# koskja/linalg-solver

Measured on AMD Instinct MI355X. Metric: fp64_lu_gflops, higher is better.
Workload: dtype f64; 1 GPU; 8192x8192 f64 LU with partial pivoting (getrf), u11 generator, resident in HBM; n=8192, nb=128, panel_mode=4, lookahead=1, parallelism=single GPU, resident_inputs=189

## Files before the change

linalg_solver_amd/csrc/common.h:

```cpp
#pragma once
#include <hip/hip_runtime.h>
#include <stdint.h>
#include <stdio.h>
#include <string>
#include <vector>

#include "../../include/lsx.h"

#ifdef LSX_TSTAMP
static __device__ long long *lsx_ts_buf;
struct TsScope {
    int id;
    __device__ void put(int tag) {
        long long *b = lsx_ts_buf;
        const int i = atomicAdd((int *)b, 1);
        if (i < (1 << 20)) { b[1 + 2 * i] = tag; b[2 + 2 * i] = wall_clock64(); }
    }
    __device__ TsScope(int id_) : id(id_) { if (lsx_ts_buf && threadIdx.x == 0 && blockIdx.x == 0 && blockIdx.y == 0) put(id); }
    __device__ ~TsScope() { if (lsx_ts_buf && threadIdx.x == 0) put(id | 0x100); }
};
#define LSX_TS(id) TsScope ts_scope_(id)
#define LSX_TS_SETTER(name) extern "C" void lsx_ts_set_##name(long long *p) { (void)hipMemcpyToSymbol(HIP_SYMBOL(lsx_ts_buf), &p, sizeof p); }
#else
#define LSX_TS(id)
#define LSX_TS_SETTER(name)
#endif

namespace lsx {

void set_error(const char *fmt, ...);

#define LSX_HIP(call)                                                                     \
    do {                                                                                  \
        hipError_t e_ = (call);                                                           \
        if (e_ != hipSuccess) {                                                           \
            lsx::set_error("%s failed: %s (%s:%d)", #call, hipGetErrorString(e_), __FILE__, \
                           __LINE__);                                                     \
            return LSX_ERR_HIP;                                                           \
        }                                                                                 \
    } while (0)

#define LSX_TRY(call)              \
    do {                           \
        int r_ = (call);           \
        if (r_ != LSX_OK) return r_; \
    } while (0)

#define LSX_ARG(cond)                                                     \
    do {                                                                  \
        if (!(cond)) {                                                    \
            lsx::set_error("bad argument: %s (%s:%d)", #cond, __FILE__, __LINE__); \
            return LSX_ERR_ARG;                                           \
        }                                                                 \
    } while (0)

struct ProfEvent {
    hipEvent_t a, b;
    int bucket;
};

struct Prof {
    unsigned mask = 0;
    int sample = 1;
    long long seen[LSX_PROF_NBUCKETS] = {0};
    std::vector<ProfEvent> pending;
    std::vector<hipEvent_t> pool;
    double ms[LSX_PROF_NBUCKETS] = {0};
    long long launches[LSX_PROF_NBUCKETS] = {0};
    double flops[LSX_PROF_NBUCKETS] = {0};
    double bytes[LSX_PROF_NBUCKETS] = {0};
};

}

struct DevBuf { void *p = nullptr; size_t bytes = 0; };

struct lsx_handle_s {
    int device = 0;
    int num_cu = 256;
    hipStream_t own_stream = nullptr;
    hipStream_t stream = nullptr;
    hipStream_t side_stream = nullptr;
    hipEvent_t ev_panel = nullptr, ev_next = nullptr, ev_start = nullptr, ev_done = nullptr;
    lsx::Prof prof;
    int nb = 128;
    int kblock = 1;
    int panel_mode = 4;
    int lookahead = 1;
    int lookahead_min = 0;
    int panel_rt = 4;
    int panel_nt = 0;
    int trsv_mode = 2;
    int gemm_stagger = 0;
    int gemm_waves = 0;
    int getri_pairs = 1;
    int left_per_step = 1;
    int chain_fused = 1;
    int chain_wait_limit = 1 << 21;
    int x_events = 0;
    int panel_debug = 0;
    int getri_plain = 0;
    int rref_first_fast = 1;
    int rref_blocked = 1;
    int getrs_t_blocked_min = 64;
    int gesvdj_max_sweeps = 30;
    int syevj_max_sweeps = 60;
    int potrs_few_max = 0;
    int lauum_descending = 0;
    int potri_order = 0;
    int gemm_no_tiles32 = 0;
    int gemm_queue_test = 0;
    int xrows_limit = 0;
    int hybrid_off = 0;
    int panel_spin_limit = 1 << 20;
    int spin_limit = 1 << 20;
    int rref_first_used = 0;
    int gecon_solves = 0;
    int gerfs_steps = 0;
    int gerfs_solves = 0;
    int getrs_t_path = 0;
    int potrs_path = 0;
    int potri_tiles = 0;
    int pocon_solves = 0;
    int porfs_steps = 0;
    int porfs_solves = 0;
    int gesvdj_sweeps = 0;
    int gesvdj_rotations = 0;
    int syevj_sweeps = 0;
    int syevj_rotations = 0;
    int panel_fallbacks = 0;
    DevBuf staging;
    DevBuf tinv;
    DevBuf rhs_work;
    DevBuf mixed_resid;
    DevBuf getri_work;
    DevBuf rref_first;
    DevBuf cond;
    DevBuf refine;
    DevBuf equil;
    DevBuf qr_work;
    DevBuf svd_work;
    DevBuf eig_work;
    DevBuf xchg;
    unsigned xchg_epoch = 0;
    DevBuf moves_all;
    DevBuf scratch;
    void *moves_buf[2] = {nullptr, nullptr};
    void *moves_api = nullptr;
    bool moves_api_valid = false;
    int *dev_status = nullptr;
};

namespace lsx {

struct OnStream {
    lsx_handle_t h; hipStream_t keep;
    OnStream(lsx_handle_t h_, hipStream_t s) : h(h_), keep(h_->stream) { h->stream = s; }
    ~OnStream() { h->stream = keep; }
};

struct GemmPlan {
    int kshift = 0;
    bool mfma_only = false;
    int *col0_static = nullptr;
    int *counters = nullptr;
    const int *avoid_word = nullptr;
    int *pass_word = nullptr;
    int *col0 = nullptr;
};
struct GemmDone {
    bool queued = false;
    bool col0_complete = false;
    int col0_tiles = 0;
};

struct PanelArgs {
    int mode, nt, rt;
    void *list;
    void *area; size_t area_bytes; bool cleared = false;
    int *xcc_word = nullptr;
    bool listed = false;
    PanelArgs(lsx_handle_t h, void *list_) : mode(h->panel_mode), nt(h->panel_nt), rt(h->panel_rt), list(list_), area(h->scratch.p), area_bytes(h->scratch.bytes) {}
};

int reserve(lsx_handle_t h, DevBuf &b, size_t need, bool *fresh = nullptr);
struct Carver {
    char *base;
    size_t off = 0;
    explicit Carver(void *b) : base((char *)b) {}
    template <typename U> U *take(size_t count) {
        off = (off + 255) & ~(size_t)255;
        U *p = base ? (U *)(base + off) : nullptr;
        off += count * sizeof(U);
        return p;
    }
};
template <class F> size_t carve_bytes(F &&layout) {
    Carver count(nullptr);
    layout(count);
    return count.off;
}
template <class F> int carve(lsx_handle_t h, DevBuf &b, F &&layout, bool *fresh = nullptr) {
    LSX_TRY(reserve(h, b, carve_bytes(layout), fresh));
    Carver c(b.p);
    layout(c);
    return LSX_OK;
}
template <class F> int carve_in(void *area, size_t bytes, const char *who, F &&layout) {
    Carver c(area);
    layout(c);
    if (area && c.off <= bytes) return LSX_OK;
    set_error("%s: needs %zu bytes of scratch, was handed %zu", who, c.off, bytes);
    return LSX_ERR_INTERNAL;
}
template <class F> size_t max_over_heights(int m, bool every, F &&bytes) {
    size_t need = 0;
    for (int mm = m; mm > 0; mm = (mm - 1) / 64 * 64) {
        const size_t b = bytes(mm);
        if (every && !b) return 0;
        if (b > need) need = b;
    }
    return need;
}
int ensure_getrf_workspace(lsx_handle_t h, int n, size_t elem);
int panel_xcd_first(lsx_handle_t h, int m, int jb, double *P, int ldp, int row0, int col0, int32_t *d_ipiv, int *d_info, double tol,
                    PanelArgs &pa);
template <typename T>
int launch_gather_pivot_cols(lsx_handle_t h, int m, int r, int row_lo, const T *src, int lds, const int32_t *d_pivots, T *dst, int ldd);
template <typename T>
int launch_rref_finish(lsx_handle_t h, int m, int bar, T *W, int ldw, const int32_t *d_pivots, int rank);
template <typename T>
int rref_blocked(lsx_handle_t h, int m, int n, int bar, T *W, int ldw, int32_t *d_pivots, int *d_rank, double tol, int pivot_rule);

struct ProfScope {
    lsx_handle_t h;
    hipStream_t st;
    int idx = -1;
    ProfScope(lsx_handle_t h_, int bucket, double flops = 0, double bytes = 0);
    ~ProfScope();
};

template <typename T>
struct Real;
template <>
struct Real<double> {
    static constexpr double eps = 2.220446049250313e-16;
};
template <>
struct Real<float> {
    static constexpr float eps = 1.1920929e-07f;
};

template <typename T>
__device__ __forceinline__ T fast_recip(T x) {
    if (sizeof(T) == 8) {
        double r = __builtin_amdgcn_rcp((double)x);
        r = r * (2.0 - (double)x * r);
        r = r * (2.0 - (double)x * r);
        return (T)r;
    }
    float r = __builtin_amdgcn_rcpf((float)x);
    r = r * (2.0f - (float)x * r);
    return (T)r;
}

template <typename T>
struct PivotRecip {
    T c, rinv;
    __device__ __forceinline__ T apply(T a) const { return (a * c) * rinv; }
};
template <typename T>
__device__ __forceinline__ PivotRecip<T> pivot_recip(T p) {
    const T safmin = sizeof(T) == 8 ? (T)0x1p-1022 : (T)0x1p-126f;
    const T c = (p < T(0) ? -p : p) < safmin ? (sizeof(T) == 8 ? (T)0x1p64 : (T)0x1p32f) : T(1);
    return PivotRecip<T>{c, fast_recip<T>(p * c)};
}


template <typename T>
int launch_fill(lsx_handle_t h, int kind, uint64_t seed, int m, int n, T *A, int lda, int row_off,
                int col_off);
template <typename T>
int launch_gemm_sub(lsx_handle_t h, int m, int n, int k, const T *A, int lda, const T *B, int ldb,
                    T *C, int ldc, const GemmPlan &plan = GemmPlan(), GemmDone *done = nullptr);
template <typename T>
int launch_gemm_acc(lsx_handle_t h, int plus, int m, int n, int k, const T *A, int lda, const T *B, int ldb,
                    T *C, int ldc, const GemmPlan &plan = GemmPlan(), GemmDone *done = nullptr);
template <typename T>
int launch_gemm_tn_acc(lsx_handle_t h, int mode, int m, int n, int k, const T *A, int lda, const T *B, int ldb, T *C,
                       int ldc, int bucket = LSX_PROF_GEMM);
template <typename T>
int launch_syrk_tn_sub(lsx_handle_t h, int n, int k, const T *A, int lda, T *C, int ldc);
template <typename T>
int launch_gemm_tn_sub(lsx_handle_t h, int m, int n, int k, const T *A, int lda, const T *B, int ldb, T *C, int ldc);
template <typename T>
int launch_lauum_tn(lsx_handle_t h, int n, const T *V, int ldv, T *C, int ldc, int order, bool descending);
int launch_rref_trace(lsx_handle_t h, int m, int n, int bar, double *R, int ldr, unsigned char *Tm,
                      int32_t *d_pivots, int32_t *d_steps, int max_steps, double *d_snaps,
                      unsigned char *d_snap_t, int max_snaps, int *d_out);
template <typename T>
int launch_panel(lsx_handle_t h, int m, int jb, T *P, int ldp, int row0, int32_t *d_ipiv,
                 int *d_info, PanelArgs &pa);
size_t panel_scratch_bytes(lsx_handle_t h, int mode, int nt, int rt, int m, size_t elem);
size_t panel_pipe_area_bytes(lsx_handle_t h, int mode, int nt, int rt, int m, bool for_driver = true);
size_t panel_x_area_bytes(lsx_handle_t h, int mode, int m, size_t elem, bool for_driver = true);
template <typename T>
int launch_laswp(lsx_handle_t h, int ncols, T *A, int lda, int row0, int jb, const int32_t *d_ipiv);
template <typename T>
int launch_laswp_moves(lsx_handle_t h, const int2 *moves, int ncols, T *A, int lda, int row0);
template <typename T>
int launch_laswp_left_all(lsx_handle_t h, T *A, int lda, int k0, int nb, int nsteps, const void *lists);
int launch_gate(lsx_handle_t h, const int *word, int target);
int launch_wait_count(lsx_handle_t h, const int *word, int target, int *info);
int launch_resid_mixed(lsx_handle_t h, int n, int nrhs, const float *A, int lda, const float *B, int ldb, const double *X,
                       int ldx, float *R, int ldr);
int launch_refine_apply(lsx_handle_t h, int n, int nrhs, int init, const float *D, int ldd, double *X, int ldx, float *Xf,
                        int ldf, double *d_out2);
template <typename T>
int diag_chain_head(lsx_handle_t h, int jb, const T *Tm, int ldt, T *Tinv, int ncols, T *A, int lda, int row0,
                    const void *moves);
template <typename T>
int launch_laswp_moves_around(lsx_handle_t h, const int2 *moves, int n, T *A, int lda, int row0, int hole_at, int hole_w);
template <typename T>
int launch_trtri(lsx_handle_t h, int lower, int jb, const T *Tm, int ldt, T *Tinv);
template <typename T>
int launch_chain_head(lsx_handle_t h, const int2 *moves, int *info, int jb, const T *Tm, int ldt, T *Tinv, int ncols, T *A,
                      int lda, int row0, const int *wait_word = nullptr, int wait_target = 0);
// ... 149 lines not shown
```

linalg_solver_amd/csrc/kernels_panel_x.hip:

```cpp
#include <algorithm>
#include <type_traits>

#include "common.h"
#include "panel_xchg.h"

namespace lsx {

constexpr int PX_WC = 8;
constexpr int PX_NT = 64 * (128 / PX_WC);
constexpr int PX_REC = 128;
constexpr int PX_NONE = 0x7fffffff;
#ifndef LSX_PX_SEG
#define LSX_PX_SEG -1
#endif
#define PX_MARK(k)                                                                  \
    if (LSX_PX_SEG >= 0) {                                                          \
        if (LSX_PX_SEG == (k)) seg_t0 = __builtin_amdgcn_s_memtime();               \
        if (LSX_PX_SEG + 1 == (k)) seg_acc += __builtin_amdgcn_s_memtime() - seg_t0; \
    }

__device__ __forceinline__ int argmax64_fast(unsigned khi, unsigned klo, int idx) {
    const unsigned mhi = rows_max_u32<4>(row16_max_u32(khi), 0);
    const bool top = (khi == mhi) & (idx != PX_NONE);
    const unsigned long long mask = __builtin_amdgcn_ballot_w64(top);
    if (mask == 0ull) return PX_NONE;
    if ((mask & (mask - 1ull)) == 0ull)
        return __builtin_amdgcn_readlane(idx, __builtin_amdgcn_readfirstlane(__builtin_ctzll(mask)));
    const unsigned mlo = rows_max_u32<4>(row16_max_u32(top ? klo : 0u), 0);
    return rows_min_i32<4>(row16_min_i32((top & (klo == mlo)) ? idx : PX_NONE), 0);
}

template <typename T>
__device__ __forceinline__ unsigned long long value_bits(T v) {
    if (sizeof(T) == 8) return (unsigned long long)__double_as_longlong((double)v);
    return (unsigned long long)__float_as_uint((float)v);
}
template <typename T>
__device__ __forceinline__ T bits_value(unsigned lo, unsigned hi) {
    if (sizeof(T) == 8) return (T)__longlong_as_double((long long)(((unsigned long long)hi << 32) | lo));
    return (T)__uint_as_float(lo);
}

template <typename T, int RT, bool DBG, bool XCD, bool FIRST = false>
__device__ __forceinline__ void panel_x_body(const int G, const int g, int m, int jb, T *__restrict__ P, int ldp,
                                             int row0, int col0, int32_t *__restrict__ ipiv,
                                             int *__restrict__ info, char *rec, XGran *far, int *status,
                                             unsigned long long *dbg, int2 *__restrict__ moves, const int spin_limit,
                                             const double tol = -1.0) {
    constexpr int NT = PX_NT, WC = PX_WC;
    constexpr int NW = NT / 64;
    constexpr int RB = 64 * RT;
    constexpr int NONE = PX_NONE;
    __shared__ T s_l[2][RB];
    __shared__ __attribute__((aligned(16))) int4 s_info[2];
    __shared__ int s_cl2;
    __shared__ int s_hist[PC_COLS], s_topid[PC_COLS], s_postop[PC_COLS];
    __shared__ int s_order[RB];
    __shared__ __attribute__((aligned(16))) T s_stage[NW][WC];

    if (info && *info < 0) return;
    const int tid = threadIdx.x, lane = tid & 63, wave = tid >> 6;
    const int base = g * RB;
    const int c0 = WC * wave;
    const bool has_cols = c0 < jb;
    const int nown = (jb + WC - 1) / WC;

    unsigned long long seg[8] = {0, 0, 0, 0, 0, 0, 0, 0};
    unsigned long long seg_t0 = 0, seg_acc = 0;
    unsigned long long tlast = 0;
#define STAMP(i)                                                              \
    if (DBG && LSX_PX_SEG < 0) {                                              \
        const unsigned long long tn_ = __builtin_amdgcn_s_memrealtime();      \
        seg[i] += tn_ - tlast;                                                \
        tlast = tn_;                                                          \
    }

    const __amdgpu_buffer_rsrc_t r_rec = __builtin_amdgcn_make_buffer_rsrc(rec, 0, 2 * G * PX_REC, 0x00020000);
    const __amdgpu_buffer_rsrc_t r_far =
        __builtin_amdgcn_make_buffer_rsrc(far, 0, 4 * G * PC_COLS * (int)sizeof(XGran), 0x00020000);
#define d_rec r_rec
#define d_far r_far

    T a[RT][WC];
    typedef T v2t __attribute__((ext_vector_type(2)));
    const bool wide = (jb == PC_COLS) && ((size_t)P % 16 == 0) && (ldp % 2 == 0);
    if (wide) {
#pragma unroll
        for (int r = 0; r < RT; ++r) {
            const int gi = base + 64 * r + lane;
            const T *src = P + (size_t)(gi < m ? gi : 0) * ldp + c0;
#pragma unroll
            for (int c = 0; c < WC; c += 2) {
                const v2t v = *(const v2t *)(src + c);
                a[r][c] = gi < m ? v[0] : T(0);
                a[r][c + 1] = gi < m ? v[1] : T(0);
            }
        }
    } else {
#pragma unroll
        for (int r = 0; r < RT; ++r) {
            const int gi = base + 64 * r + lane;
            const T *src = P + (size_t)gi * ldp + c0;
#pragma unroll
            for (int c = 0; c < WC; ++c) a[r][c] = (gi < m && c0 + c < jb) ? src[c] : T(0);
        }
    }
    for (int t = tid; t < PC_COLS; t += NT) { s_topid[t] = t; s_postop[t] = t; }
    for (int t = tid; t < RB; t += NT) s_order[t] = -1;
    unsigned frozen = 0;
#pragma unroll
    for (int r = 0; r < RT; ++r)
        if (base + 64 * r + lane >= m) frozen |= 1u << r;
    int pos[FIRST ? RT : 1];
    if (FIRST) {
#pragma unroll
        for (int r = 0; r < RT; ++r) pos[r] = base + 64 * r + lane;
    }
    constexpr unsigned EMASK = FIRST ? 0xffu : 0x7fffffffu;
    auto track_swap = [&](const int j, const int win, const int wpos) __attribute__((always_inline)) {
        if (FIRST) {
#pragma unroll
            for (int r = 0; r < RT; ++r)
                if (pos[r] == j && base + 64 * r + lane != win) pos[r] = wpos;
        }
    };
    bool failed = false;
    u4 hA = u4{0u, 0u, 0u, 0u}, hB = u4{0u, 0u, 0u, 0u};
    __builtin_amdgcn_s_waitcnt(0x0F70);
    __syncthreads();

    auto replay = [&](int jj) __attribute__((always_inline)) {
        const int c = s_hist[jj] & 0x3fffffff;
        const bool zero_piv = (s_hist[jj] >> 30) & 1;
        const int p = (c < jb) ? s_postop[c] : c;
        const int d = s_topid[jj];
        if (p != jj) {
            s_topid[jj] = c;
            if (p < jb) s_topid[p] = d;
            s_postop[d] = p;
            if (c < jb) s_postop[c] = jj;
        }
        if (g == 0) {
            ipiv[jj] = row0 + p;
            if (zero_piv && info && *info == 0) *info = col0 + jj + 1;
        }
    };

    auto shot_async = [&](u4 &h, const int jn) __attribute__((always_inline)) {
        const int off = ((jn & 1) * G + (lane < G ? lane : 0)) * PX_REC;
        asm volatile("buffer_load_dwordx4 %0, %1, %2, 0 offen sc1" : "+v"(h) : "v"(off), "s"(d_rec));
    };
    auto wait_a = [&]() __attribute__((always_inline)) { asm volatile("s_waitcnt vmcnt(1)" : "+v"(hA), "+v"(hB)); };
    auto wait_b = [&]() __attribute__((always_inline)) { asm volatile("s_waitcnt vmcnt(0)" : "+v"(hA), "+v"(hB)); };
    auto store16 = [&](const unsigned lo, const unsigned hi, const unsigned z, const unsigned w, const int off,
                       const __amdgpu_buffer_rsrc_t &desc) __attribute__((always_inline)) {
#define LSX_ST16(R0, R1, R2, R3, POL)                                                                                   \
    asm volatile("v_mov_b32 v" #R0 ", %0\n\tv_mov_b32 v" #R1 ", %1\n\tv_mov_b32 v" #R2 ", %2\n\tv_mov_b32 v" #R3 ", %3\n\t"    \
                 "buffer_store_dwordx4 v[" #R0 ":" #R3 "], %4, %5, 0 offen" POL "\n\ts_nop 1"                             \
                 : : "v"(lo), "v"(hi), "s"(z), "v"(w), "v"(off), "s"(desc) : "v" #R0, "v" #R1, "v" #R2, "v" #R3)
        if (WC == 8) {
            if (XCD) LSX_ST16(124, 125, 126, 127, ""); else LSX_ST16(124, 125, 126, 127, " sc1");
        } else {
            if (XCD) LSX_ST16(252, 253, 254, 255, ""); else LSX_ST16(252, 253, 254, 255, " sc1");
        }
#undef LSX_ST16
    };
    auto store_header = [&](const int jn, const double val, const int row, const bool neg, const int rpos = 0)
                            __attribute__((always_inline)) {
        store16((unsigned)__double2loint(val), (unsigned)__double2hiint(val),
                (unsigned)__builtin_amdgcn_readfirstlane(row),
                (unsigned)(jn + 1) | (neg ? 0x80000000u : 0u) | (FIRST ? ((unsigned)rpos << 8) : 0u),
                ((jn & 1) * G + g) * PX_REC, d_rec);
    };
    auto store_gran = [&](const __amdgpu_buffer_rsrc_t &desc, const int off, const T v, const int jn) __attribute__((always_inline)) {
        unsigned lo, hi;
        if (sizeof(T) == 8) { lo = (unsigned)__double2loint((double)v); hi = (unsigned)__double2hiint((double)v); }
        else { lo = __float_as_uint((float)v); hi = 0u; }
        store16(lo, hi, (unsigned)(jn + 1), 0u, off, desc);
    };
    auto choose_and_announce = [&](auto CNt, const int jn) __attribute__((always_inline)) -> int {
        constexpr int CN = decltype(CNt)::value;
        double nv = -1.0;
        int ni = NONE;
        int np = NONE;
#pragma unroll
        for (int r = 0; r < RT; ++r) {
            const double av = fabs((double)a[r][CN]);
            bool better;
            if (FIRST) better = (((frozen >> r) & 1u) == 0u) & (av > tol) & (pos[r] < np);
            else better = (((frozen >> r) & 1u) == 0u) & (av > nv);
            nv = better ? av : nv;
            ni = better ? base + 64 * r + lane : ni;
            if (FIRST) np = better ? pos[r] : np;
        }
        const unsigned long long kb = (ni != NONE) ? (unsigned long long)__double_as_longlong(nv) : 0ull;
        const int win = FIRST ? argmax64_fast((ni != NONE) ? (unsigned)(0x7fffffff - np) : 0u, 0u, ni)
                              : argmax64_fast((unsigned)(kb >> 32), (unsigned)kb, ni);
        const bool have = win != NONE;
        const int cl = have ? win - base : -1;
        if (have) {
            if (lane == (cl & 63)) {
                const int ck = cl >> 6;
                const int roff = ((jn & 1) * G + g) * PX_REC;
#pragma unroll
                for (int k = 0; k < RT; ++k)
                    if (ck == k) {
                        store_header(jn, fabs((double)a[k][CN]), win, a[k][CN] < T(0), FIRST ? pos[k] : 0);
#pragma unroll
                        for (int c = (CN & 7) + 1; c < 8; ++c)
                            store_gran(d_rec, roff + 16 * c, a[k][(CN & 8) + c], jn);
                    }
            }
        } else if (lane == 0) {
            store_header(jn, 0.0, -1, false);
        }
        return cl;
    };
    const unsigned stage_addr = (unsigned)(unsigned long long)(T __attribute__((address_space(3))) *)&s_stage[wave][0];
    auto publish_far = [&](auto CLOt, auto NCt, const int jn, const int cl_) __attribute__((always_inline)) {
        constexpr int CLO = decltype(CLOt)::value, NC = decltype(NCt)::value;
        const int cl = __builtin_amdgcn_readfirstlane(cl_);
        if (cl < 0 || !has_cols) return;
        if (lane == (cl & 63)) {
            const int ck = cl >> 6;
#pragma unroll
            for (int k = 0; k < RT; ++k)
                if (ck == k) {
#pragma unroll
                    for (int c = 0; c < NC; ++c) {
                        if (sizeof(T) == 8)
                            asm volatile("ds_write_b64 %0, %1 offset:%2" : : "v"(stage_addr), "v"(a[k][CLO + c]), "n"(8 * c) : "memory");
                        else
                            asm volatile("ds_write_b32 %0, %1 offset:%2" : : "v"(stage_addr), "v"(a[k][CLO + c]), "n"(4 * c) : "memory");
                    }
                }
        }
        const int q = lane & (NC - 1);
        unsigned lo, hi = 0u;
        if (sizeof(T) == 8) {
            double v;
            asm volatile("ds_read_b64 %0, %1\n\ts_waitcnt lgkmcnt(0)" : "=v"(v) : "v"(stage_addr + 8u * q) : "memory");
            lo = (unsigned)__double2loint(v); hi = (unsigned)__double2hiint(v);
        } else {
            asm volatile("ds_read_b32 %0, %1\n\ts_waitcnt lgkmcnt(0)" : "=v"(lo) : "v"(stage_addr + 4u * q) : "memory");
        }
        if (lane < NC)
            store16(lo, hi, (unsigned)(jn + 1), 0u, (((jn & 3) * G + g) * PC_COLS + c0 + CLO + q) * (int)sizeof(XGran), d_far);
    };
    auto far_update = [&](auto CLOt, auto NCt, const int j, const int bg) __attribute__((always_inline)) -> bool {
        constexpr int CLO = decltype(CLOt)::value, NC = decltype(NCt)::value;
        const int off = (((j & 3) * G + bg) * PC_COLS + c0 + CLO + (lane & (NC - 1))) * (int)sizeof(XGran);
        u4 v;
        int spins = failed ? spin_limit : 0;
        for (;;) {
            v = __builtin_amdgcn_raw_buffer_load_b128(r_far, off, opaque_zero(), 16);
            if (!__any(v.z != (unsigned)(j + 1))) break;
            if (++spins > spin_limit) return false;
        }
        T l[RT];
#pragma unroll
        for (int r = 0; r < RT; ++r) l[r] = s_l[j & 1][64 * r + lane];
        const T un = -bits_value<T>(v.x, v.y);
        asm volatile("s_nop 1" : : "v"(un));
#pragma unroll
        for (int c = 0; c < NC; ++c) {
#pragma unroll
            for (int r = 0; r < RT; ++r) {
                if (sizeof(T) == 8)
                    asm volatile("v_fmac_f64_dpp %0, %1, %2 row_newbcast:%3 row_mask:0xf bank_mask:0xf"
                                 : "+v"(a[r][CLO + c]) : "v"(un), "v"(l[r]), "n"(c));
                else
                    asm volatile("v_fmac_f32_dpp %0, %1, %2 row_newbcast:%3 row_mask:0xf bank_mask:0xf"
                                 : "+v"(a[r][CLO + c]) : "v"(un), "v"(l[r]), "n"(c));
            }
        }
        return true;
    };
    typedef std::integral_constant<int, 0> I0;
    typedef std::integral_constant<int, 8> I8;
    typedef std::integral_constant<int, WC> IWC;
    auto follow = [&](const int j, const int ow) __attribute__((always_inline)) {
        const int par = j & 1;
        const bool stamp = DBG && wave == ow + 1;
        if (stamp) tlast = __builtin_amdgcn_s_memrealtime();
        __syncthreads();
        if (stamp) STAMP(4)
        const int4 inf = s_info[par];
        const int wrow = inf.x;
        const bool act = (inf.y & 1) != 0;
        failed |= (inf.y & 2) != 0;
        const bool valid = wrow >= 0;
        const int bg = valid ? wrow / RB : 0;
        if (wave == (ow == 0 ? NW - 1 : 0) && lane == 63) {
            s_hist[j] = valid ? (wrow | (act ? 0 : (1 << 30))) : j;
            if (j > 0) replay(j - 1);
            if (valid && bg == g) s_order[wrow - base] = j;
        }
        if (valid && bg == g) {
            const int wl = wrow - base;
            if ((wl & 63) == lane) frozen |= 1u << (wl >> 6);
        }
        if (valid) track_swap(j, wrow, inf.w);
        bool ok = true;
        if (act && wave > ow && has_cols) ok = far_update(I0{}, IWC{}, j, bg);
        if (stamp) STAMP(5)
        if (!ok && !failed) {
            failed = true;
            if (lane == 0) atomicExch(status, 1);
        }
        if (j + 1 < jb) {
            if ((j & 7) < 7) {
                if (wave > ow) publish_far(I0{}, IWC{}, j + 1, inf.z);
            } else {
                const bool hand_over = (j & (WC - 1)) == WC - 1;
                if (hand_over && wave == ow + 1) {
                    __builtin_amdgcn_s_setprio(3);
                    const int cl = choose_and_announce(I0{}, j + 1);
                    if (lane == 0) s_cl2 = cl;
                    shot_async(hA, j + 1);
                }
                __syncthreads();
                const int nown_ = hand_over ? ow + 1 : ow;
                if (hand_over && wave == ow + 1) {
                    if constexpr (WC == 16) publish_far(I8{}, I8{}, j + 1, s_cl2);
                    shot_async(hB, j + 1);
                }
                else if (wave > nown_) publish_far(I0{}, IWC{}, j + 1, s_cl2);
            }
        }
        if (stamp) STAMP(6)
    };

    auto own = [&](auto CJt, const int j) __attribute__((always_inline)) {
        constexpr int CJ = decltype(CJt)::value;
        constexpr int JC = CJ & 7;
        constexpr int CB = CJ & 8;
        constexpr bool FIRSTB = WC == 16 && CJ < 8;
        constexpr bool NEAR = JC < 7;
        const int par = j & 1;
        const bool more = j + 1 < jb;
        if (DBG && CJ == 0) tlast = __builtin_amdgcn_s_memrealtime();
        PX_MARK(0)
        bool failed_now = failed;
        bool pend = lane < G;
        unsigned hlo = 0u, hhi = 0u, hneg = 0u;
        int hrow = NONE;
        int hpos = 0;
        auto absorb = [&](const u4 &h) __attribute__((always_inline)) {
            const bool ok = pend & ((h.w & EMASK) == (unsigned)(j + 1));
            hlo = ok ? h.x : hlo;
            hhi = ok ? h.y : hhi;
            hneg = ok ? (h.w >> 31) : hneg;
            if (FIRST) hpos = ok ? (int)((h.w >> 8) & 0x3fffu) : hpos;
            hrow = ok ? ((int)h.z >= 0 ? (int)h.z : NONE) : hrow;
            pend = ok ? false : pend;
        };
        constexpr bool TWO = !FIRSTB || JC == 0;
        if (TWO) wait_a(); else wait_b();
        PX_MARK(1)
        absorb(hA);
        if (__any(pend)) {
            if (TWO) { wait_b(); absorb(hB); }
            int spins = failed ? spin_limit : 0;
            while (__any(pend)) {
                if (++spins > spin_limit) { failed_now = true; break; }
                const u4 h = __builtin_amdgcn_raw_buffer_load_b128(
                    r_rec, (par * G + (lane < G ? lane : 0)) * PX_REC, opaque_zero(), 16);
                absorb(h);
            }
        }
        const bool hv = hrow != NONE;
        const int win = FIRST ? argmax64_fast(hv ? (unsigned)(0x7fffffff - hpos) : 0u, 0u, hrow)
                              : argmax64_fast(hv ? hhi : 0u, hv ? hlo : 0u, hrow);
        const bool valid = (win != NONE) & !failed_now;
        const int bg = valid ? win / RB : 0;
        const int wpos = FIRST ? __builtin_amdgcn_readlane(hpos, bg) : 0;
        const unsigned plo = (unsigned)__builtin_amdgcn_readlane((int)hlo, bg);
        const unsigned phi = (unsigned)__builtin_amdgcn_readlane((int)hhi, bg);
        const bool pneg = __builtin_amdgcn_readlane((int)hneg, bg) != 0;
        const double pabs = __longlong_as_double((long long)(((unsigned long long)phi << 32) | plo));
        PX_MARK(2)
        STAMP(0)
        const bool act = valid & (pabs != 0.0);
        const bool fetch = NEAR && more && act;
        u4 nq = u4{0u, 0u, 0u, 0u};
        const int noff = (par * G + bg) * PX_REC + 16 * (lane & 7);
        if (fetch) nq = __builtin_amdgcn_raw_buffer_load_b128(r_rec, noff, opaque_zero(), 16);
        PivotRecip<T> rinv = act ? pivot_recip<T>((T)pabs) : PivotRecip<T>{T(1), T(0)};
        if (pneg) rinv.rinv = -rinv.rinv;
        if (valid && bg == g) {
            const int wl = win - base;
            if ((wl & 63) == lane) frozen |= 1u << (wl >> 6);
        }
        if (valid) track_swap(j, win, wpos);
        T l[RT];
#pragma unroll
        for (int r = 0; r < RT; ++r) {
            const T v = rinv.apply(a[r][CJ]);
            l[r] = ((frozen >> r) & 1u) ? T(0) : v;
            s_l[par][64 * r + lane] = l[r];
            a[r][CJ] = (act & (((frozen >> r) & 1u) == 0u)) ? l[r] : a[r][CJ];
        }
        PX_MARK(3)
        wait_b();
        bool upd = false;
        if (fetch) {
            int spins = 0;
            for (;;) {
                const int q = lane & 7;
                if (!__any((q > JC) & (nq.z != (unsigned)(j + 1)))) break;
                if (++spins > spin_limit) { failed_now = true; break; }
                nq = __builtin_amdgcn_raw_buffer_load_b128(r_rec, noff, opaque_zero(), 16);
            }
            upd = !failed_now;
        }
        STAMP(1)
        PX_MARK(4)
        if (upd) {
            const T un = -bits_value<T>(nq.x, nq.y);
            asm volatile("s_nop 1" : : "v"(un));
#pragma unroll
            for (int c = JC + 1; c < 8; ++c) {
#pragma unroll
                for (int r = 0; r < RT; ++r) {
                    if (sizeof(T) == 8)
                        asm volatile("v_fmac_f64_dpp %0, %1, %2 row_newbcast:%3 row_mask:0xf bank_mask:0xf"
                                     : "+v"(a[r][CB + c]) : "v"(un), "v"(l[r]), "n"(c));
                    else
                        asm volatile("v_fmac_f32_dpp %0, %1, %2 row_newbcast:%3 row_mask:0xf bank_mask:0xf"
                                     : "+v"(a[r][CB + c]) : "v"(un), "v"(l[r]), "n"(c));
                }
            }
        }
        PX_MARK(5)
        int cl = -1;
        if (NEAR && more) cl = choose_and_announce(std::integral_constant<int, (CJ < WC - 1 ? CJ + 1 : WC - 1)>{}, j + 1);
        PX_MARK(6)
        const bool act2 = act & !failed_now;
        if (lane == 0) s_info[par] = make_int4(valid ? win : -1, (act2 ? 1 : 0) | (failed_now ? 2 : 0), cl, wpos);
        if (failed_now && !failed) {
            failed = true;
            if (lane == 0) atomicExch(status, 1);
        }
        if (NEAR && more) shot_async(hA, j + 1);
        STAMP(2)
        PX_MARK(7)
        __syncthreads();
        if (!FIRSTB && NEAR && more) shot_async(hB, j + 1);
        PX_MARK(8)
        STAMP(3)
        if constexpr (FIRSTB) { if (more) {
            bool ok = true;
            if (act2) ok = far_update(I8{}, I8{}, j, bg);
            if (!ok && !failed) {
                failed = true;
                if (lane == 0) atomicExch(status, 1);
            }
            if (NEAR) {
                publish_far(I8{}, I8{}, j + 1, cl);
            } else {
                const int cl8 = choose_and_announce(I8{}, j + 1);
                if (lane == 0) s_cl2 = cl8;
                shot_async(hA, j + 1);
                __syncthreads();
                shot_async(hB, j + 1);
            }
            STAMP(7)
        } } else if (!NEAR && more) {
            __syncthreads();
        }
    };

    if (wave == 0) {
        __builtin_amdgcn_s_setprio(3);
        const int cl = choose_and_announce(I0{}, 0);
        if (lane == 0) s_cl2 = cl;
        shot_async(hA, 0);
    }
    __syncthreads();
    if (wave == 0) {
        if constexpr (WC == 16) publish_far(I8{}, I8{}, 0, s_cl2);
        shot_async(hB, 0);
    }
    else publish_far(I0{}, IWC{}, 0, s_cl2);

    for (int ow = 0; ow < nown; ++ow) {
        const int j0 = WC * ow;
        if (wave == ow) {
#define COL(k) if constexpr (k < WC) { if (j0 + k < jb) own(std::integral_constant<int, k>{}, j0 + k); }
            COL(0) COL(1) COL(2) COL(3) COL(4) COL(5) COL(6) COL(7)
            COL(8) COL(9) COL(10) COL(11) COL(12) COL(13) COL(14) COL(15)
#undef COL
            __builtin_amdgcn_s_setprio(0);
        } else {
            for (int k = 0; k < WC; ++k)
                if (j0 + k < jb) follow(j0 + k, ow);
        }
    }
    if (DBG && lane == 0)
        for (int i = 0; i < 8; ++i) atomicAdd(&dbg[g * 16 + i], seg[i]);
    if (DBG && LSX_PX_SEG >= 0 && lane == 0) atomicAdd(&dbg[g * 16 + 12], seg_acc);
#undef STAMP
#undef d_rec
#undef d_far
    __syncthreads();
    if (tid == NT - 1) replay(jb - 1);
    if (failed && info && lane == 0) atomicMin(info, -0x40000000);
    __syncthreads();
    if (g == 0 && moves) {
        for (int t = tid; t < 2 * PC_COLS; t += NT) {
            int dst = -1, src = -1;
            if (t < jb) {
                dst = t;
                src = s_hist[t] & 0x3fffffff;
            } else if (t >= PC_COLS && t - PC_COLS < jb) {
                const int d = t - PC_COLS;
                bool is_pivot = false;
                for (int q = 0; q < jb; ++q) is_pivot |= ((s_hist[q] & 0x3fffffff) == d);
                if (!is_pivot) { dst = s_postop[d]; src = d; }
            }
            if (dst == src) dst = src = -1;
            moves[t] = make_int2(dst, src);
        }
    }
    if (has_cols) {
#pragma unroll
        for (int r = 0; r < RT; ++r) {
            const int lr = 64 * r + lane;
            const int gi = base + lr;
            if (gi < m) {
                const int ord = s_order[lr];
                const int dest = ord >= 0 ? ord : (gi < jb ? s_postop[gi] : gi);
                T *dst = P + (size_t)dest * ldp + c0;
                if (wide) {
#pragma unroll
                    for (int c = 0; c < WC; c += 2) {
                        v2t v;
                        v[0] = a[r][c]; v[1] = a[r][c + 1];
                        *(v2t *)(dst + c) = v;
                    }
                } else {
#pragma unroll
                    for (int c = 0; c < WC; ++c)
                        if (c0 + c < jb) dst[c] = a[r][c];
                }
            }
        }
    }
}

template <typename T, int RT, bool DBG, bool FIRST = false>
__global__ __launch_bounds__(PX_NT, PX_NT / 256) void panel_x_kernel(int m, int jb, T *__restrict__ P, int ldp, int row0, int col0,
                                                        int32_t *__restrict__ ipiv, int *__restrict__ info,
                                                        char *rec, XGran *far, int *status, unsigned long long *dbg,
                                                        int2 *__restrict__ moves, int *xcc, int *xcc_word,
                                                        int spin_limit, double tol) {
    if (blockIdx.x & 7) return;
    LSX_TS(1);
    const int G = gridDim.x >> 3, g = blockIdx.x >> 3;
    if (spin_limit < 0) {
        spin_limit = -spin_limit;
        if (g == G - 1 && G > 1)
            for (int i = 0; i < 900; ++i) __builtin_amdgcn_s_sleep(127);
    }
    __shared__ int s_same;
    if (threadIdx.x < 64) {
        unsigned id;
        asm volatile("s_getreg_b32 %0, hwreg(HW_REG_XCC_ID, 0, 4)" : "=s"(id));
        const int lane = threadIdx.x;
        if (lane == 0) {
            __hip_atomic_store(&xcc[g], (int)id + 1, __ATOMIC_RELAXED, __HIP_MEMORY_SCOPE_AGENT);
            if (g == 0 && xcc_word) __hip_atomic_store(xcc_word, (int)id + 1, __ATOMIC_RELAXED, __HIP_MEMORY_SCOPE_AGENT);
        }
        bool pend = lane < G, same = true;
        int spins = 0;
        while (__any(pend)) {
            const int v = __hip_atomic_load(&xcc[lane < G ? lane : 0], __ATOMIC_RELAXED, __HIP_MEMORY_SCOPE_AGENT);
            if (pend && v != 0) { pend = false; same = v == (int)id + 1; }
            if (++spins > spin_limit) { same = false; break; }
        }
        const bool all_same = !__any(!same);
        if (lane == 0) {
            s_same = all_same ? 1 : 0;
            if (DBG && dbg) dbg[g * 16 + 15] = ((unsigned long long)id << 8) | (all_same ? 1u : 0u);
        }
    }
    __syncthreads();
    if (s_same)
        panel_x_body<T, RT, DBG, true, FIRST>(G, g, m, jb, P, ldp, row0, col0, ipiv, info, rec, far, status, dbg, moves, spin_limit, tol);
    else
        panel_x_body<T, RT, DBG, false, FIRST>(G, g, m, jb, P, ldp, row0, col0, ipiv, info, rec, far, status, dbg, moves, spin_limit, tol);
}

struct XArea {
    int *status, *xcc; char *rec; XGran *far; unsigned long long *dbg = nullptr;
    size_t bytes;
    void lay(Carver &c, int G, bool debug) {
        status = c.take<int>(64), xcc = status + 16;
        rec = c.take<char>((size_t)2 * G * PX_REC);
        far = c.take<XGran>((size_t)4 * G * PC_COLS);
        if (debug) dbg = c.take<unsigned long long>((size_t)G * 16);
        bytes = c.off;
    }
};
struct XShape { int rt, G; };
static XShape x_shape(lsx_handle_t h, int m, size_t elem) {
    const int rt = m <= 32 * 64 * 1 ? 1 : m <= 32 * 64 * 2 ? 2 : (elem == 4 && m > 32 * 64 * 4) ? 8 : 4;
    const int G = (m + 64 * rt - 1) / (64 * rt);
    return {rt, (G > 32 || G > h->num_cu) ? 0 : G};
}

size_t panel_x_area_bytes(lsx_handle_t h, int mode, int m, size_t elem, bool for_driver) {
    if (mode != 4 || (for_driver && (h->panel_debug || h->nb > PC_COLS))) return 0;
    m = std::min(m, 32 * 64 * (elem == 8 ? 4 : 8));
    const size_t need = max_over_heights(m, for_driver, [&](int mm) {
        const int G = x_shape(h, mm, elem).G;
        return G ? carve_bytes([&](Carver &c) { XArea().lay(c, G, h->panel_debug); }) : (size_t)0;
    });
    return (need + 255) & ~(size_t)255;
}

template <typename T, int RT>
static int panel_xcd_rt(lsx_handle_t h, int m, int jb, T *P, int ldp, int row0, int col0, int32_t *d_ipiv, int *d_info,
                        PanelArgs &pa, const double first_tol = -1.0) {
    const int G = x_shape(h, m, sizeof(T)).G;
    if (jb > PC_COLS || G == 0) return 1;
    XArea a;
    LSX_TRY(carve_in(pa.area, pa.area_bytes, "panel_xcd", [&](Carver &c) { a.lay(c, G, h->panel_debug); }));
    if (!pa.cleared) LSX_HIP(hipMemsetAsync(a.status, 0, a.bytes, h->stream));
    if (first_tol >= 0.0) {
        if constexpr (sizeof(T) == 8 && RT <= 4)
            hipLaunchKernelGGL((panel_x_kernel<T, RT, false, true>), dim3(8 * G), dim3(PX_NT), 0, h->stream, m, jb, P, ldp, row0,
                               col0, d_ipiv, d_info, a.rec, a.far, a.status, a.dbg, (int2 *)pa.list, a.xcc, pa.xcc_word, h->panel_spin_limit, first_tol);
        else
            return 1;
    } else if (h->panel_debug)
        hipLaunchKernelGGL((panel_x_kernel<T, RT, true>), dim3(8 * G), dim3(PX_NT), 0, h->stream, m, jb, P, ldp, row0,
                           col0, d_ipiv, d_info, a.rec, a.far, a.status, a.dbg, (int2 *)pa.list, a.xcc, pa.xcc_word, h->panel_spin_limit, -1.0);
    else
        hipLaunchKernelGGL((panel_x_kernel<T, RT, false>), dim3(8 * G), dim3(PX_NT), 0, h->stream, m, jb, P, ldp, row0,
                           col0, d_ipiv, d_info, a.rec, a.far, a.status, a.dbg, (int2 *)pa.list, a.xcc, pa.xcc_word, h->panel_spin_limit, -1.0);
    LSX_HIP(hipGetLastError());
    pa.listed = true;
    return LSX_OK;
}

template <typename T>
int panel_xcd(lsx_handle_t h, int m, int jb, T *P, int ldp, int row0, int col0, int32_t *d_ipiv, int *d_info, PanelArgs &pa) {
    const int rt = x_shape(h, m, sizeof(T)).rt;
    if (rt == 1) return panel_xcd_rt<T, 1>(h, m, jb, P, ldp, row0, col0, d_ipiv, d_info, pa);
    if (rt == 2) return panel_xcd_rt<T, 2>(h, m, jb, P, ldp, row0, col0, d_ipiv, d_info, pa);
    if (rt == 8) return panel_xcd_rt<T, sizeof(T) == 4 ? 8 : 4>(h, m, jb, P, ldp, row0, col0, d_ipiv, d_info, pa);
    return panel_xcd_rt<T, 4>(h, m, jb, P, ldp, row0, col0, d_ipiv, d_info, pa);
}

int panel_xcd_first(lsx_handle_t h, int m, int jb, double *P, int ldp, int row0, int col0, int32_t *d_ipiv, int *d_info,
                    double tol, PanelArgs &pa) {
    pa.listed = false;
    if (tol < 0.0 || m > 32 * 64 * 4) return 1;
    if (m <= 32 * 64 * 1) return panel_xcd_rt<double, 1>(h, m, jb, P, ldp, row0, col0, d_ipiv, d_info, pa, tol);
    if (m <= 32 * 64 * 2) return panel_xcd_rt<double, 2>(h, m, jb, P, ldp, row0, col0, d_ipiv, d_info, pa, tol);
    return panel_xcd_rt<double, 4>(h, m, jb, P, ldp, row0, col0, d_ipiv, d_info, pa, tol);
}

template int panel_xcd<double>(lsx_handle_t, int, int, double *, int, int, int, int32_t *, int *, PanelArgs &);
template int panel_xcd<float>(lsx_handle_t, int, int, float *, int, int, int, int32_t *, int *, PanelArgs &);

}

LSX_TS_SETTER(panelx)
```

Baseline: 22690 GFLOP/s.

## Stage panel tile loads/stores through LDS and overlap load with XCC handshake

```diff
diff --git a/linalg_solver_amd/csrc/common.h b/linalg_solver_amd/csrc/common.h
--- a/linalg_solver_amd/csrc/common.h
+++ b/linalg_solver_amd/csrc/common.h
@@ -11,18 +11,23 @@
 static __device__ long long *lsx_ts_buf;
 struct TsScope {
     int id;
-    __device__ void put(int tag) {
+    __device__ static void put_at(int tag, long long t) {
         long long *b = lsx_ts_buf;
         const int i = atomicAdd((int *)b, 1);
-        if (i < (1 << 20)) { b[1 + 2 * i] = tag; b[2 + 2 * i] = wall_clock64(); }
+        if (i < (1 << 20)) { b[1 + 2 * i] = tag; b[2 + 2 * i] = t; }
     }
+    __device__ void put(int tag) { put_at(tag, wall_clock64()); }
     __device__ TsScope(int id_) : id(id_) { if (lsx_ts_buf && threadIdx.x == 0 && blockIdx.x == 0 && blockIdx.y == 0) put(id); }
     __device__ ~TsScope() { if (lsx_ts_buf && threadIdx.x == 0) put(id | 0x100); }
 };
 #define LSX_TS(id) TsScope ts_scope_(id)
+#define LSX_TS_MARK(id, k, t) do { if (lsx_ts_buf && blockIdx.x == 0) TsScope::put_at((id) | 0x200 | ((k) << 12), (long long)(t)); } while (0)
+#define LSX_TS_MARKS 1
 #define LSX_TS_SETTER(name) extern "C" void lsx_ts_set_##name(long long *p) { (void)hipMemcpyToSymbol(HIP_SYMBOL(lsx_ts_buf), &p, sizeof p); }
 #else
 #define LSX_TS(id)
+#define LSX_TS_MARK(id, k, t)
+#define LSX_TS_MARKS 0
 #define LSX_TS_SETTER(name)
 #endif
 
diff --git a/linalg_solver_amd/csrc/kernels_panel_x.hip b/linalg_solver_amd/csrc/kernels_panel_x.hip
--- a/linalg_solver_amd/csrc/kernels_panel_x.hip
+++ b/linalg_solver_amd/csrc/kernels_panel_x.hip
@@ -41,24 +41,111 @@
     return (T)__uint_as_float(lo);
 }
 
+enum { PX_PLAIN = 0, PX_WIDE = 1, PX_STAGED = 2 };
+__device__ __forceinline__ unsigned px_mov(const unsigned x) {
+    unsigned y;
+    asm("v_mov_b32 %0, %1" : "=v"(y) : "v"(x));
+    return y;
+}
+__device__ __forceinline__ double px_own_reg(const double v) {
+    return __hiloint2double((int)px_mov((unsigned)__double2hiint(v)), (int)px_mov((unsigned)__double2loint(v)));
+}
+__device__ __forceinline__ float px_own_reg(const float v) { return __uint_as_float(px_mov(__float_as_uint(v))); }
+template <typename T>
+struct PxImg {
+    static constexpr int EPV = 16 / (int)sizeof(T);
+    static constexpr int LPR = PC_COLS / EPV;
+    static constexpr int RPI = 64 / LPR;
+    static constexpr int NI = 64 / ((PX_NT / 64) * RPI);
+    static constexpr int ROWB = PC_COLS * (int)sizeof(T) + 16;
+    static constexpr int BYTES = 64 * ROWB;
+    typedef T vec __attribute__((ext_vector_type(EPV)));
+};
+template <typename T>
+__device__ __forceinline__ int px_tile_mode(const int jb, const T *P, const int ldp) {
+    if (jb != PC_COLS || (size_t)P % 16 != 0 || ldp % 2 != 0) return PX_PLAIN;
+    return (ldp * sizeof(T)) % 16 == 0 ? PX_STAGED : PX_WIDE;
+}
+template <typename T, int RT>
+__device__ __forceinline__ void px_load_tile(T (&a)[RT][PX_WC], const int mode, char *img, const T *__restrict__ P,
+                                             const int ldp, const int m, const int jb, const int base) {
+    constexpr int WC = PX_WC, NW = PX_NT / 64;
+    typedef PxImg<T> I;
+    typedef typename I::vec vec;
+    typedef T v2t __attribute__((ext_vector_type(2)));
+    const int lane = threadIdx.x & 63, wave = threadIdx.x >> 6, c0 = WC * wave;
+    if (mode == PX_STAGED) {
+        const int sub = lane / I::LPR, piece = lane % I::LPR;
+        vec t[I::NI];
+        auto issue = [&](const int r) __attribute__((always_inline)) {
+#pragma unroll
+            for (int i = 0; i < I::NI; ++i) {
+                const int gi = base + 64 * r + (i * NW + wave) * I::RPI + sub;
+                t[i] = *(const vec *)(P + (size_t)(gi < m ? gi : 0) * ldp + I::EPV * piece);
+                if (gi >= m) t[i] = vec{};
+            }
+        };
+        issue(0);
+#pragma unroll
+        for (int r = 0; r < RT; ++r) {
+            if (r > 0) __syncthreads();
+#pragma unroll
+            for (int i = 0; i < I::NI; ++i)
+                *(vec *)(img + ((i * NW + wave) * I::RPI + sub) * I::ROWB + 16 * piece) = t[i];
+            __syncthreads();
+            if (r + 1 < RT) issue(r + 1);
+#pragma unroll
+            for (int k = 0; k < WC / I::EPV; ++k) {
+                const vec v = *(const vec *)(img + lane * I::ROWB + (c0 + I::EPV * k) * (int)sizeof(T));
+#pragma unroll
+                for (int e = 0; e < I::EPV; ++e) a[r][I::EPV * k + e] = v[e];
+            }
+        }
+    } else if (mode == PX_WIDE) {
+#pragma unroll
+        for (int r = 0; r < RT; ++r) {
+            const int gi = base + 64 * r + lane;
+            const T *src = P + (size_t)(gi < m ? gi : 0) * ldp + c0;
+#pragma unroll
+            for (int c = 0; c < WC; c += 2) {
+                const v2t v = *(const v2t *)(src + c);
+                a[r][c] = gi < m ? v[0] : T(0);
+                a[r][c + 1] = gi < m ? v[1] : T(0);
+            }
+        }
+    } else {
+#pragma unroll
+        for (int r = 0; r < RT; ++r) {
+            const int gi = base + 64 * r + lane;
+            const T *src = P + (size_t)gi * ldp + c0;
+#pragma unroll
+            for (int c = 0; c < WC; ++c) a[r][c] = (gi < m && c0 + c < jb) ? src[c] : T(0);
+        }
+    }
+}
+
+#define PX_TMARK(k) if (PX_TM) tm[k] = __builtin_amdgcn_s_memrealtime();
+
 template <typename T, int RT, bool DBG, bool XCD, bool FIRST = false>
 __device__ __forceinline__ void panel_x_body(const int G, const int g, int m, int jb, T *__restrict__ P, int ldp,
                                              int row0, int col0, int32_t *__restrict__ ipiv,
                                              int *__restrict__ info, char *rec, XGran *far, int *status,
                                              unsigned long long *dbg, int2 *__restrict__ moves, const int spin_limit,
+                                             unsigned long long (&tm)[7], T (&a)[RT][PX_WC], const int tmode, char *img,
                                              const double tol = -1.0) {
     constexpr int NT = PX_NT, WC = PX_WC;
     constexpr int NW = NT / 64;
     constexpr int RB = 64 * RT;
     constexpr int NONE = PX_NONE;
+#define PX_TM (DBG || LSX_TS_MARKS)
     __shared__ T s_l[2][RB];
     __shared__ __attribute__((aligned(16))) int4 s_info[2];
     __shared__ int s_cl2;
     __shared__ int s_hist[PC_COLS], s_topid[PC_COLS], s_postop[PC_COLS];
+    __shared__ int s_mark[PC_COLS];
     __shared__ int s_order[RB];
     __shared__ __attribute__((aligned(16))) T s_stage[NW][WC];
 
-    if (info && *info < 0) return;
     const int tid = threadIdx.x, lane = tid & 63, wave = tid >> 6;
     const int base = g * RB;
     const int c0 = WC * wave;
@@ -81,31 +168,8 @@
 #define d_rec r_rec
 #define d_far r_far
 
-    T a[RT][WC];
     typedef T v2t __attribute__((ext_vector_type(2)));
-    const bool wide = (jb == PC_COLS) && ((size_t)P % 16 == 0) && (ldp % 2 == 0);
-    if (wide) {
-#pragma unroll
-        for (int r = 0; r < RT; ++r) {
-            const int gi = base + 64 * r + lane;
-            const T *src = P + (size_t)(gi < m ? gi : 0) * ldp + c0;
-#pragma unroll
-            for (int c = 0; c < WC; c += 2) {
-                const v2t v = *(const v2t *)(src + c);
-                a[r][c] = gi < m ? v[0] : T(0);
-                a[r][c + 1] = gi < m ? v[1] : T(0);
-            }
-        }
-    } else {
-#pragma unroll
-        for (int r = 0; r < RT; ++r) {
-            const int gi = base + 64 * r + lane;
-            const T *src = P + (size_t)gi * ldp + c0;
-#pragma unroll
-            for (int c = 0; c < WC; ++c) a[r][c] = (gi < m && c0 + c < jb) ? src[c] : T(0);
-        }
-    }
-    for (int t = tid; t < PC_COLS; t += NT) { s_topid[t] = t; s_postop[t] = t; }
+    for (int t = tid; t < PC_COLS; t += NT) { s_topid[t] = t; s_postop[t] = t; s_mark[t] = 0; }
     for (int t = tid; t < RB; t += NT) s_order[t] = -1;
     unsigned frozen = 0;
 #pragma unroll
@@ -476,6 +540,7 @@
         const int cl = choose_and_announce(I0{}, 0);
         if (lane == 0) s_cl2 = cl;
         shot_async(hA, 0);
+        PX_TMARK(3)
     }
     __syncthreads();
     if (wave == 0) {
@@ -497,6 +562,7 @@
                 if (j0 + k < jb) follow(j0 + k, ow);
         }
     }
+    PX_TMARK(4)
     if (DBG && lane == 0)
         for (int i = 0; i < 8; ++i) atomicAdd(&dbg[g * 16 + i], seg[i]);
     if (DBG && LSX_PX_SEG >= 0 && lane == 0) atomicAdd(&dbg[g * 16 + 12], seg_acc);
@@ -506,8 +572,67 @@
     __syncthreads();
     if (tid == NT - 1) replay(jb - 1);
     if (failed && info && lane == 0) atomicMin(info, -0x40000000);
-    __syncthreads();
-    if (g == 0 && moves) {
+    const bool list = g == 0 && moves;
+    if (list)
+        for (int t = tid; t < jb; t += NT) {
+            const int c = s_hist[t] & 0x3fffffff;
+            if (c < PC_COLS) s_mark[c] = 1;
+        }
+    auto dest_of = [&](const int lr) __attribute__((always_inline)) -> int {
+        const int gi = base + lr, ord = s_order[lr];
+        return ord >= 0 ? ord : (gi < jb ? s_postop[gi] : gi);
+    };
+    if (tmode == PX_STAGED) {
+        typedef PxImg<T> I;
+        typedef typename I::vec vec;
+        const int sub = lane / I::LPR, piece = lane % I::LPR;
+#pragma unroll
+        for (int r = 0; r < RT; ++r) {
+            if (r > 0) __syncthreads();
+#pragma unroll
+            for (int k = 0; k < WC / I::EPV; ++k) {
+                vec v;
+#pragma unroll
+                for (int e = 0; e < I::EPV; ++e) v[e] = px_own_reg(a[r][I::EPV * k + e]);
+                *(vec *)(img + lane * I::ROWB + (c0 + I::EPV * k) * (int)sizeof(T)) = v;
+            }
+            __syncthreads();
+#pragma unroll
+            for (int i = 0; i < I::NI; ++i) {
+                const int sr = (i * NW + wave) * I::RPI + sub;
+                if (base + 64 * r + sr < m) {
+                    int dest = dest_of(64 * r + sr);
+                    asm volatile("" : "+v"(dest));
+                    *(vec *)(P + (size_t)dest * ldp + I::EPV * piece) = *(const vec *)(img + sr * I::ROWB + 16 * piece);
+                }
+            }
+        }
+    } else {
+        __syncthreads();
+        if (has_cols) {
+#pragma unroll
+            for (int r = 0; r < RT; ++r) {
+                const int lr = 64 * r + lane;
+                if (base + lr < m) {
+                    T *dst = P + (size_t)dest_of(lr) * ldp + c0;
+                    if (tmode == PX_WIDE) {
+#pragma unroll
+                        for (int c = 0; c < WC; c += 2) {
+                            v2t v;
+                            v[0] = a[r][c]; v[1] = a[r][c + 1];
+                            *(v2t *)(dst + c) = v;
+                        }
+                    } else {
+#pragma unroll
+                        for (int c = 0; c < WC; ++c)
+                            if (c0 + c < jb) dst[c] = a[r][c];
+                    }
+                }
+            }
+        }
+    }
+    PX_TMARK(5)
+    if (list) {
         for (int t = tid; t < 2 * PC_COLS; t += NT) {
             int dst = -1, src = -1;
             if (t < jb) {
@@ -515,38 +640,24 @@
                 src = s_hist[t] & 0x3fffffff;
             } else if (t >= PC_COLS && t - PC_COLS < jb) {
                 const int d = t - PC_COLS;
-                bool is_pivot = false;
-                for (int q = 0; q < jb; ++q) is_pivot |= ((s_hist[q] & 0x3fffffff) == d);
-                if (!is_pivot) { dst = s_postop[d]; src = d; }
+                if (!s_mark[d]) { dst = s_postop[d]; src = d; }
             }
             if (dst == src) dst = src = -1;
             moves[t] = make_int2(dst, src);
         }
     }
-    if (has_cols) {
-#pragma unroll
-        for (int r = 0; r < RT; ++r) {
-            const int lr = 64 * r + lane;
-            const int gi = base + lr;
-            if (gi < m) {
-                const int ord = s_order[lr];
-                const int dest = ord >= 0 ? ord : (gi < jb ? s_postop[gi] : gi);
-                T *dst = P + (size_t)dest * ldp + c0;
-                if (wide) {
-#pragma unroll
-                    for (int c = 0; c < WC; c += 2) {
-                        v2t v;
-                        v[0] = a[r][c]; v[1] = a[r][c + 1];
-                        *(v2t *)(dst + c) = v;
-                    }
-                } else {
-#pragma unroll
-                    for (int c = 0; c < WC; ++c)
-                        if (c0 + c < jb) dst[c] = a[r][c];
-                }
-            }
-        }
-    }
+    if (PX_TM) {
+        __builtin_amdgcn_s_waitcnt(0x0F70);
+        PX_TMARK(6)
+        if (tid == 0) {
+            if (DBG && dbg) {
+                const int slot[7] = {0, 8, 9, 10, 11, 13, 14};
+                for (int k = 1; k < 7; ++k) dbg[g * 16 + slot[k]] = tm[k] - tm[0];
+            }
+            for (int k = 0; k < 7; ++k) LSX_TS_MARK(1, k, tm[k]);
+        }
+    }
+#undef PX_TM
 }
 
 template <typename T, int RT, bool DBG, bool FIRST = false>
@@ -557,6 +668,9 @@
                                                         int spin_limit, double tol) {
     if (blockIdx.x & 7) return;
     LSX_TS(1);
+#define PX_TM (DBG || LSX_TS_MARKS)
+    unsigned long long tm[7] = {0, 0, 0, 0, 0, 0, 0};
+    PX_TMARK(0)
     const int G = gridDim.x >> 3, g = blockIdx.x >> 3;
     if (spin_limit < 0) {
         spin_limit = -spin_limit;
@@ -564,14 +678,21 @@
             for (int i = 0; i < 900; ++i) __builtin_amdgcn_s_sleep(127);
     }
     __shared__ int s_same;
+    __shared__ __attribute__((aligned(16))) char s_img[PxImg<T>::BYTES];
+    unsigned id;
+    asm volatile("s_getreg_b32 %0, hwreg(HW_REG_XCC_ID, 0, 4)" : "=s"(id));
+    if (threadIdx.x == 0) {
+        __hip_atomic_store(&xcc[g], (int)id + 1, __ATOMIC_RELAXED, __HIP_MEMORY_SCOPE_AGENT);
+        if (g == 0 && xcc_word) __hip_atomic_store(xcc_word, (int)id + 1, __ATOMIC_RELAXED, __HIP_MEMORY_SCOPE_AGENT);
+    }
+    const int info_v = info ? *info : 0;
+    T a[RT][PX_WC];
+    const int tmode = px_tile_mode(jb, P, ldp);
+    px_load_tile<T, RT>(a, tmode, s_img, P, ldp, m, jb, g * 64 * RT);
+    if (PX_TM) __builtin_amdgcn_s_waitcnt(0x0F70);
+    PX_TMARK(2)
     if (threadIdx.x < 64) {
-        unsigned id;
-        asm volatile("s_getreg_b32 %0, hwreg(HW_REG_XCC_ID, 0, 4)" : "=s"(id));
         const int lane = threadIdx.x;
-        if (lane == 0) {
-            __hip_atomic_store(&xcc[g], (int)id + 1, __ATOMIC_RELAXED, __HIP_MEMORY_SCOPE_AGENT);
-            if (g == 0 && xcc_word) __hip_atomic_store(xcc_word, (int)id + 1, __ATOMIC_RELAXED, __HIP_MEMORY_SCOPE_AGENT);
-        }
         bool pend = lane < G, same = true;
         int spins = 0;
         while (__any(pend)) {
@@ -586,10 +707,21 @@
         }
     }
     __syncthreads();
-    if (s_same)
-        panel_x_body<T, RT, DBG, true, FIRST>(G, g, m, jb, P, ldp, row0, col0, ipiv, info, rec, far, status, dbg, moves, spin_limit, tol);
-    else
-        panel_x_body<T, RT, DBG, false, FIRST>(G, g, m, jb, P, ldp, row0, col0, ipiv, info, rec, far, status, dbg, moves, spin_limit, tol);
+    PX_TMARK(1)
+#undef PX_TM
+    __builtin_amdgcn_s_waitcnt(0x0F70);
+    if (__builtin_amdgcn_readfirstlane(info_v) < 0) {
+        if (g == 0 && moves)
+            for (int t = threadIdx.x; t < 2 * PC_COLS; t += PX_NT) moves[t] = make_int2(-1, -1);
+        return;
+    }
+    if (__builtin_amdgcn_readfirstlane(s_same)) {
+        panel_x_body<T, RT, DBG, true, FIRST>(G, g, m, jb, P, ldp, row0, col0, ipiv, info, rec, far, status, dbg, moves, spin_limit, tm, a, tmode, s_img, tol);
+    } else {
+        T a2[RT][PX_WC];
+        px_load_tile<T, RT>(a2, tmode, s_img, P, ldp, m, jb, g * 64 * RT);
+        panel_x_body<T, RT, DBG, false, FIRST>(G, g, m, jb, P, ldp, row0, col0, ipiv, info, rec, far, status, dbg, moves, spin_limit, tm, a2, tmode, s_img, tol);
+    }
 }
 
 struct XArea {
```

After: 22910 GFLOP/s (median of 6 runs). +1.0%, better.
